# TAdeJong/pyGPA

Hardware: AMD Instinct MI355X
Metric: Mpixels/s displacement-field extraction (3 peaks, 4096^2 img) + achieved HBM GB/s (higher is better)
Workload: dtype f32; 1 GPU; 4096x4096 synthetic hex moire, 3 Bragg peaks x 16 k-vectors, sigma=10, weighted DCT-PCG unwrap kmax=10, image resident in HBM, u downloaded to pinned host memory inside the step (BASELINE.json configs[2]); x_planes=12, d2h_of_u=included, overlapped with the next step (copy stream), images_in_flight=1

## Files before the change

pygpa_amd/csrc/gpa_api.hip:

```cpp
#include "gpa_plan.h"

static thread_local std::string g_err;
int gpa_fail(int code, const std::string& msg) {
  g_err = msg;
  return code;
}
namespace gpa {
static const char* const kOptNames[OPT_COUNT] = {
    "PBS_FULLBAND", "SERIAL_UNWRAP", "NO_WORKER", "NO_KSPLIT", "NO_COMPACT", "NO_SHARED",
    "NO_PAIR", "TRI_SMALL", "TRI_Q", "NO_MR", "MR_FORCE_BLUESTEIN", "NO_ROWPQ", "COLSOLVE", "NO_LAT",
    "F32_EPS_FLOOR", "COLSTREAM_CHUNK", "NO_ROWHALF", "PAIR_MAXSIDE", "ROWHALF_MINLG", "NO_PQDCT",
    "NO_REORDER", "NO_RAW", "NO_TILEFUSE", "NO_ROWPERS", "NO_LFTILE", "LF_ALL_ROUNDS", "DFT_ENGINE", "GAUSS_FFT_MINR", "NO_GAUSS2D", "NO_DFT_HALF", "F32_STALL", "PBS_LDS_PAD", "NO_SHARED_PHASES", "PA_STAG", "PA_STAG_TICKS", "PA_ROT", "LF_STACK_BYTES", "NO_YSPEC", "YSPEC_GROUP", "NO_PB_SKIP"};
static OptVal g_opts[OPT_COUNT];
static std::once_flag g_opts_once;
static void opt_assign(OptVal& o, const char* value) {
  o.set = value != nullptr;
  o.num = value ? atof(value) : 0.0;
  memset(o.str, 0, sizeof(o.str));
  if (value) strncpy(o.str, value, sizeof(o.str) - 1);
}
static void opts_from_env() {
  for (int k = 0; k < OPT_COUNT; ++k) opt_assign(g_opts[k], getenv((std::string("GPA_") + kOptNames[k]).c_str()));
}
const OptVal& opt(OptKey k) {
  std::call_once(g_opts_once, opts_from_env);
  return g_opts[k];
}
}

Axis make_axis(int n) {
  Axis a;
  a.n = n;
  int lg = 0;
  while ((1 << lg) < n) ++lg;
  if ((1 << lg) == n) {
    a.padded = false;
  } else {
    lg = 0;
    while ((1 << lg) < 2 * n - 1) ++lg;
    a.padded = true;
  }
  if (lg < 6) {
    lg = 6;
    a.padded = ((1 << lg) != n);
  }
  a.lg = lg;
  a.L = 1 << lg;
  a.extL = a.padded ? n - 1 : 0;
  a.extR = 0;
  return a;
}

Axis compact_axis(const Axis& full, int E) {
  if (!full.padded || E >= (full.n - 1) / 2) return full;
  int lg = 6;
  while ((1 << lg) < full.n + 2 * E) ++lg;
  if (lg >= full.lg) return full;
  Axis a = full;
  a.lg = lg;
  a.L = 1 << lg;
  a.extL = a.extR = E;
  return a;
}

int upload_real_table(gpa_plan* p, void* dst, const std::vector<double>& v) {
  if (p->dtype == GPA_F32) HIP_TRY(upload_as<float>(dst, v, p->stream));
  else HIP_TRY(upload_as<double>(dst, v, p->stream));
  return GPA_OK;
}

int plan_reserve(gpa_plan* p, DevBuf& b, size_t bytes, const char* what) {
  const hipError_t e = b.reserve(bytes, p->stream);
  if (e != hipSuccess) return fail(GPA_ERR_HIP, std::string(what) + "(" + std::to_string(bytes) + "): " + hipGetErrorString(e));
  return GPA_OK;
}

int dmalloc(gpa_plan* p, void** ptr, size_t bytes) {
  DevBuf b(&p->ws_bytes);
  TRY(plan_reserve(p, b, bytes, "hipMalloc"));
  *ptr = b.ptr;
  p->owned.push_back(std::move(b));
  return GPA_OK;
}
int plan_build(gpa_plan* p) {
  HIP_TRY(hipSetDevice(p->device));
  HIP_TRY(hipStreamCreateWithFlags(&p->stream, hipStreamNonBlocking));
  HIP_TRY(hipEventCreate(&p->ev0));
  HIP_TRY(hipEventCreate(&p->ev1));
  for (auto& e : p->stage_ev) HIP_TRY(hipEventCreate(&e));
  const size_t npx = (size_t)p->n0 * p->n1;
  const int B = p->max_batch;
  TRY(dmalloc(p, &p->tw0, (size_t)p->ax0.L * p->csz));
  TRY(upload_twiddles(p, p->tw0, p->ax0.L));
  TRY(dmalloc(p, &p->tw1, (size_t)p->ax1.L * p->csz));
  TRY(upload_twiddles(p, p->tw1, p->ax1.L));
// ... 236 lines not shown
```

pygpa_amd/csrc/gpa_api_driver.hip:

```cpp
#include "gpa_plan.h"

struct ExtractOut {
  void* lockins;
  int32_t* kidx;
  void* grads;
  void* absw;
  int grad_mode;
};

static int check_ranges(gpa_plan* p, const std::string& fn, int P, int K, int kmax) {
  if (P < 2 || P > p->max_peaks) return fail(GPA_ERR_STATE, fn + ": need 2 <= P <= 8");
  if (K < 1 || P * K > p->max_batch) return fail(GPA_ERR_STATE, fn + ": P*K exceeds max_batch");
  if (kmax < 1) return fail(GPA_ERR_ARG, "kmax must be >= 1");
  return GPA_OK;
}

static int extract_stage(gpa_plan* p, const double* kvecs, int P, const double* klists, int K, double sigma, int* Bx, int passb) {
  TRY(stage_sweep(p, kvecs, P, klists, K, sigma, Bx, passb));
  TRY(stage_kmat(p, kvecs, P));
  {
    const size_t side = opt_set(OPT_PAIR_MAXSIDE) ? (size_t)opt(OPT_PAIR_MAXSIDE).num : 1024;
    p->use_pair = (size_t)p->n0 * p->n1 <= side * side && !opt_set(OPT_NO_PAIR);
  }
  if (p->use_pair && !p->have_uwp) {
// ... 185 lines not shown
                                         void* u, void* lockins, int32_t* kidx) {
  return extract_enqueue(p, "gpa_extract_displacement_field", image, kvecs, P, klists, K, sigma, mask_border, kmax, u,
                         {lockins, kidx, nullptr, nullptr, 0});
}

int gpa_extract_displacement_field_grad_async(gpa_plan* p, const void* image, const double* kvecs, int P,
                                              const double* klists, int K, double sigma, int mask_border, int kmax,
                                              int grad_mode, void* u, void* lockins, int32_t* kidx, void* grads, void* absw) {
  return extract_enqueue(p, "gpa_extract_displacement_field_grad_async", image, kvecs, P, klists, K, sigma, mask_border, kmax, u,
                         {lockins, kidx, grads, absw, grad_mode});
}

static int ensure_batch_unwrap(gpa_plan* p, int B) {
  if (B <= p->uwb_images) {
    if (!unwrap_set_active(&p->uwb, 2 * B)) return fail(GPA_ERR_STATE, "batched unwrap workspace: bad active count");
    return GPA_OK;
  }
  HIP_TRY(hipStreamSynchronize(p->stream));
  if (p->uwb_images) unwrap_workspace_destroy(&p->uwb);
  p->uwb_images = 0;
  p->uwb_bytes = 0;
  size_t bb = 0;
  hipError_t e = unwrap_workspace_create(p->dtype, p->n0, p->n1, p->stream, &p->uwb, &bb, 2 * B);
  if (e != hipSuccess) {
    unwrap_workspace_destroy(&p->uwb);
    return fail(GPA_ERR_HIP, std::string("batched unwrap workspace: ") + hipGetErrorString(e));
  }
  if (!unwrap_supports_batch(&p->uwb)) {
    unwrap_workspace_destroy(&p->uwb);
    return fail(GPA_ERR_STATE, "gpa_extract_displacement_field_batch: this image shape has no batched unwrap");
  }
  e = p->d_wnorm_b.reserve((size_t)B * p->n0 * p->n1 * p->rsz, p->stream);
  if (e == hipSuccess) e = p->h_iters_b.reserve((size_t)8 * B * sizeof(int), p->stream);
  if (e != hipSuccess) {
    unwrap_workspace_destroy(&p->uwb);
    return fail(GPA_ERR_HIP, std::string("batched driver buffers: ") + hipGetErrorString(e));
  }
  p->uwb_images = B;
  p->uwb_bytes = bb;
  return GPA_OK;
}

static int ensure_batch_sweep(gpa_plan* p, int chunk, size_t t_img, size_t l_img) {
  TRY(plan_reserve(p, p->bT, (size_t)chunk * t_img, "batched sweep buffers"));
  TRY(plan_reserve(p, p->bL, (size_t)chunk * l_img, "batched sweep buffers"));
  TRY(plan_reserve(p, p->bMean, (size_t)chunk * 8, "batched sweep buffers"));
  return plan_reserve(p, p->bScratch, (size_t)chunk * 1024 * sizeof(double), "batched sweep buffers");
}

static int read_batch_iters(gpa_plan* p, int B, int* iters_out) {
  HIP_TRY(hipStreamSynchronize(p->stream));
  for (int j = 0; j < 2 * B; ++j) iters_out[j] = p->h_iters_b.as<int>()[4 * j + unwrap_iters_slot(&p->uwb)];
  return GPA_OK;
}

int gpa_extract_displacement_field_batch_dev(gpa_plan* p, const void* images, int B, const double* kvecs, int P,
                                             const double* klists, int K, double sigma, int mask_border, int kmax,
                                             void* u, int* iters_out) {
  const char* fn = "gpa_extract_displacement_field_batch";
  if (!p || !images || !kvecs || !klists || !u) return fail(GPA_ERR_ARG, std::string(fn) + ": null argument");
  if (B < 1 || B > 4096) return fail(GPA_ERR_ARG, std::string(fn) + ": need 1 <= images <= 4096");
  TRY(check_ranges(p, fn, P, K, kmax));
  HIP_TRY(hipSetDevice(p->device));
  int Bx = 0;
  TRY(extract_stage(p, kvecs, P, klists, K, sigma, &Bx, SWEEP_PASSB_SELECT));
  TRY(ensure_batch_unwrap(p, B));
  const size_t npx = (size_t)p->n0 * p->n1;
  const size_t t_img = (size_t)Bx * npx * p->csz, l_img = (size_t)P * npx * p->csz;
  const int chunk = (int)std::min<size_t>((size_t)B, std::max<size_t>(1, ((size_t)3 << 30) / t_img));
  TRY(ensure_batch_sweep(p, chunk, t_img, l_img));
  int nparts = 0;
  const size_t rstride = 2 * npx;
  const size_t pstride = (size_t)(unwrap_partials_buffer(&p->uwb, 2) - unwrap_partials_buffer(&p->uwb, 0));
  for (int c0 = 0; c0 < B; c0 += chunk) {
    const int nimg = std::min(chunk, B - c0);
    const void* image = (const char*)images + (size_t)c0 * npx * p->rsz;
    HIP_TRY(launch_mean(p->dtype, image, npx, p->bScratch.as<double>(), p->bMean.ptr, p->stream, nimg));
    TRY(run_passA(p, image, p->bMean.ptr, p->bT.ptr, Bx, nimg));
    TRY(passB_select(p, {p->bT.ptr, nimg, Bx}, P, K, p->bL.ptr, nullptr, true));
    HIP_TRY(launch_reconstruct_setup(p->dtype, p->bL.ptr, p->d_kmat, P, p->n0, p->n1, mask_border,
                                     p->d_wnorm_b.as<char>() + (size_t)c0 * npx * p->rsz,
                                     unwrap_residual_buffer(&p->uwb, 2 * c0), unwrap_residual_buffer(&p->uwb, 2 * c0 + 1),
                                     unwrap_partials_buffer(&p->uwb, 2 * c0), unwrap_partials_buffer(&p->uwb, 2 * c0 + 1),
                                     &nparts, p->stream, nimg, rstride, pstride, p->lk_raw ? p->d_ystep : nullptr));
  }
  hipError_t e = unwrap_enqueue_prepared(&p->uwb, p->d_wnorm_b.ptr, nparts, kmax, 1e-9, true, u, p->stream);
  if (e == hipSuccess) e = unwrap_fetch_iters(&p->uwb, p->h_iters_b.as<int>(), p->stream);
  if (e != hipSuccess) return fail(GPA_ERR_HIP, std::string("batched unwrap: ") + hipGetErrorString(e));
  return iters_out ? read_batch_iters(p, B, iters_out) : GPA_OK;
}

int gpa_supports_batch(gpa_plan* p) {
  if (!p) return 0;
  return unwrap_supports_batch(&p->uw) ? 1 : 0;
}

int gpa_last_batch_iters(gpa_plan* p, int B, int* iters_out) {
  if (!p || !iters_out || B < 1 || B > p->uwb_images) return fail(GPA_ERR_ARG, "gpa_last_batch_iters: bad argument");
  return read_batch_iters(p, B, iters_out);
}

int gpa_extract_gradients(gpa_plan* p, const void* image, const double* kvecs, int P, const double* klists, int K,
                          double sigma, int mask_border, void* dudx, void* dudy, void* wnorm) {
  if (!p || !image || !kvecs || !klists || !dudx || !dudy || !wnorm)
    return fail(GPA_ERR_ARG, "gpa_extract_gradients: null argument");
  TRY(check_ranges(p, "gpa_extract_gradients", P, K, 1));
  HIP_TRY(hipSetDevice(p->device));
  const size_t npx = (size_t)p->n0 * p->n1;
  HIP_TRY(hipMemcpyAsync(p->d_image, image, npx * p->rsz, hipMemcpyHostToDevice, p->stream));
  TRY(sweep_peaks_dev(p, p->d_image, nullptr, kvecs, P, klists, K, sigma, p->d_lockin, nullptr, true));
  TRY(stage_kmat(p, kvecs, P));
  HIP_TRY(launch_reconstruct(p->dtype, p->d_lockin, p->d_kmat, P, p->n0, p->n1, mask_border, p->d_dudx, p->d_dudy,
                             p->d_wnorm, p->stream, p->lk_raw ? p->d_ystep : nullptr));
  HIP_TRY(hipMemcpyAsync(dudx, p->d_dudx, (size_t)2 * p->n0 * (p->n1 - 1) * p->rsz, hipMemcpyDeviceToHost, p->stream));
  HIP_TRY(hipMemcpyAsync(dudy, p->d_dudy, (size_t)2 * (p->n0 - 1) * p->n1 * p->rsz, hipMemcpyDeviceToHost, p->stream));
  HIP_TRY(hipMemcpyAsync(wnorm, p->d_wnorm, npx * p->rsz, hipMemcpyDeviceToHost, p->stream));
  HIP_TRY(hipStreamSynchronize(p->stream));
  return GPA_OK;
}
```

pygpa_amd/csrc/gpa_internal.h:

```cpp
#pragma once
#include <hip/hip_runtime.h>
#include <stdint.h>

#include "gpa_devbuf.h"
#include "gpa_fft.h"
#include "gpa_mrfft.h"

#ifndef GPA_F64_WAVES
#define GPA_F64_WAVES 2
#endif

namespace gpa {

struct KernelProfiler {
  struct Rec { const char* name; hipEvent_t a, b; };
  static constexpr int MAXREC = 4096;
  Rec rec[MAXREC];
  int n = 0;
  hipEvent_t pool[2 * MAXREC];
  int npool = 0;
};
extern thread_local KernelProfiler* g_kprof;
struct ProfScope {
  hipStream_t s;
  KernelProfiler::Rec* r = nullptr;
  ProfScope(const char* name, hipStream_t stream) : s(stream) {
    KernelProfiler* k = g_kprof;
    if (!k || k->n >= KernelProfiler::MAXREC) return;
    for (int j = 0; j < 2; ++j)
      if (k->npool < 2 * (k->n + 1)) { if (hipEventCreate(&k->pool[k->npool]) != hipSuccess) return; ++k->npool; }
    r = &k->rec[k->n];
    r->name = name;
    r->a = k->pool[2 * k->n];
    r->b = k->pool[2 * k->n + 1];
    ++k->n;
    (void)hipEventRecord(r->a, s);
  }
  ~ProfScope() { if (r) (void)hipEventRecord(r->b, s); }
};
#if defined(__HIPCC__)
__device__ __forceinline__ int xcd_tile(int b, int grid) {
  const int base = grid >> 3, rem = grid & 7, x = b & 7, idx = b >> 3;
  return x * base + (x < rem ? x : rem) + idx;
}
#endif

inline hipError_t set_dynamic_lds_once(const void* kern, int bytes, unsigned& done) {
  int dev = 0;
  (void)hipGetDevice(&dev);
  const unsigned bit = 1u << (dev & 31);
  if (done & bit) return hipSuccess;
  hipError_t e = hipFuncSetAttribute(kern, hipFuncAttributeMaxDynamicSharedMemorySize, bytes);
  if (e == hipSuccess) done |= bit;
  return e;
}

inline int device_cus() {
  static int n[32] = {};
  int dev = 0;
  (void)hipGetDevice(&dev);
  int& slot = n[dev & 31];
  if (!slot) {
    int cus = 0;
    if (hipDeviceGetAttribute(&cus, hipDeviceAttributeMultiprocessorCount, dev) != hipSuccess || cus <= 0) cus = 256;
    slot = cus;
  }
  return slot;
}

enum OptKey {
  OPT_PBS_FULLBAND, OPT_SERIAL_UNWRAP, OPT_NO_WORKER, OPT_NO_KSPLIT, OPT_NO_COMPACT, OPT_NO_SHARED,
  OPT_NO_PAIR, OPT_TRI_SMALL, OPT_TRI_Q, OPT_NO_MR, OPT_MR_FORCE_BLUESTEIN, OPT_NO_ROWPQ,
  OPT_COLSOLVE, OPT_NO_LAT, OPT_F32_EPS_FLOOR, OPT_COLSTREAM_CHUNK, OPT_NO_ROWHALF, OPT_PAIR_MAXSIDE, OPT_ROWHALF_MINLG, OPT_NO_PQDCT,
  OPT_NO_REORDER, OPT_NO_RAW, OPT_NO_TILEFUSE, OPT_NO_ROWPERS, OPT_NO_LFTILE, OPT_LF_ALL_ROUNDS, OPT_DFT_ENGINE, OPT_GAUSS_FFT_MINR, OPT_NO_GAUSS2D, OPT_NO_DFT_HALF, OPT_F32_STALL, OPT_PBS_LDS_PAD, OPT_NO_SHARED_PHASES, OPT_PA_STAG, OPT_PA_STAG_TICKS, OPT_PA_ROT, OPT_LF_STACK_BYTES, OPT_NO_YSPEC, OPT_YSPEC_GROUP, OPT_NO_PB_SKIP, OPT_COUNT
};
struct OptVal {
  bool set;
  double num;
  char str[24];
};
const OptVal& opt(OptKey k);
inline bool opt_set(OptKey k) { return opt(k).set; }

#define GPA_PROF_CAT2(a, b) a##b
#define GPA_PROF_CAT(a, b) GPA_PROF_CAT2(a, b)
#define GPA_PROF(name, stream) ::gpa::ProfScope GPA_PROF_CAT(_gpa_prof_, __LINE__)(name, stream)

struct Axis {
  int n;
  int lg;
  int L;
  bool padded;
  int extL, extR;
};
inline int axis_tpf(const Axis& a) { return a.L / 16; }

GPA_HD int axis_src(int m, int n, int L, bool padded, int extL, int extR) {
  if (!padded) return m;
  if (m < n) return m;
  if (m < n + extR) return m - n;
  if (m >= L - extL) return m - L + n;
  return -1;
}

struct SweepTables {
  void* cxb;
  void* sx;
  void* wxw;
  void* wxr;
  void* cyb;
  void* sy;
  void* wyw;
  void* wyr;
  void* dx;
  void* dy;
  int* planeof;
};

hipError_t launch_tables(int dtype, const Axis& a0, const Axis& a1, const double* kl,
                         const double* kr, int B, const double* pw, int Bx, const SweepTables& tb,
                         hipStream_t s);
hipError_t launch_mean(int dtype, const void* image, size_t count, double* scratch,
                       void* mean_out, hipStream_t s, int nimg = 1);
hipError_t launch_passA(int dtype, const Axis& a0, int n1, const void* image, const void* mean,
                        const SweepTables& tb, const void* Hx, const void* tw0, void* Tbuf,
                        int Bx, hipStream_t s, int nimg = 1);
struct PassAYspec {
  void* Yhat;
  void* strips;
  const int* groups;
  const int* planes;
  int ngroups;
  unsigned blockmask;
  int E, Epad;
};
hipError_t launch_passA_yspec(int dtype, const Axis& a0, const Axis& a1, const void* image, const void* mean,
                              const SweepTables& tb, const void* Hx, const void* tw0, const void* tw1, void* Tbuf, int Bx,
                              const PassAYspec& ys, hipStream_t s, int nimg = 1);
hipError_t launch_passB(int dtype, const Axis& a1, int n0, const void* Tbuf, const void* Hy,
                        const void* tw1, const SweepTables& tb, int P, int K, bool select,
                        void* out, int32_t* kidx, hipStream_t s, int nimg = 1, int Bx = 0);
hipError_t launch_passB_ext(int dtype, const Axis& a1, int n0, const void* Tbuf, const void* Hy, const void* tw1,
                            const SweepTables& tb, int K, int mode, void* out, int32_t* kidx, const uint8_t* gate,
                            void* psi, hipStream_t s, int P = 1);
hipError_t launch_passB_split(int dtype, const Axis& a1, int n0, const void* Tbuf, const void* Hy, const void* tw1,
                              const SweepTables& tb, int P, int K, int ksplit, void* part, int32_t* pidx, void* out,
                              int32_t* kidx, hipStream_t s);
hipError_t launch_phasegrad(int dtype, const void* psi, int K, const int32_t* kidx, int n0, int n1, const double* kl,
                            const double* kr, int mode, void* grad, hipStream_t s, const double* ystep = nullptr, int P = 1);
int passA_cols(int dtype, int lg);
int spec_index_rt(int lg, int tid, int reg, int elems = 16);

hipError_t launch_reconstruct(int dtype, const void* lockin, const double* kmat ,
                              int P, int n0, int n1, int border, void* dudx, void* dudy,
                              void* wnorm, hipStream_t s, const double* ystep = nullptr );

hipError_t launch_reconstruct_tile(int dtype, const void* lockin, const double* kmat, int P, int n0, int n1, int border,
                                   int i0, int j0, int t0, int t1, void* const dx[2], size_t dx_pitch, void* const dy[2],
                                   size_t dy_pitch, void* const wn[2], size_t wn_pitch, hipStream_t s,
                                   const double* ystep = nullptr);
hipError_t launch_reconstruct_setup(int dtype, const void* lockin, const double* kmat, int P, int n0, int n1,
                                    int border, void* wnorm, void* r0, void* r1, double* part0, double* part1,
                                    int* nparts, hipStream_t s, int nimg = 1, size_t rstride = 0, size_t pstride = 0,
                                    const double* ystep = nullptr );

hipError_t launch_prediff(int dtype, const void* grads, const void* w, const double* kmat, int P, int n0, int n1,
                          void* dudx, void* dudy, void* wnorm, hipStream_t s);

hipError_t launch_wlstsq(int dtype, const void* b, const void* w, const double* kmat, int P, size_t npx,
                         void* out, hipStream_t s);

hipError_t launch_jacobian(int dtype, const void* grads, const void* w, const double* kmat, int P, size_t npx,
                           double nmperpixel, const double* dks , void* J, hipStream_t s);
hipError_t launch_cabs(int dtype, const void* z, size_t count, void* out, hipStream_t s);
hipError_t launch_props(int dtype, const void* jac, size_t npx, int add_identity, double refangle, double refscale,
                        int diff, void* out, hipStream_t s);

struct KerelskyArgs {
  double a0[4], x0[4], retry_cost;
  int max_nfev, has_a0;
};
hipError_t launch_kerelsky(int dtype, const void* jac, size_t npx, const KerelskyArgs& p, void* out, double* cost, hipStream_t s);

hipError_t launch_field_jacobian(int dtype, int nimg, int n0, int n1, const void* u, double nmperpixel, int add_identity, void* J,
                                 void* props, double refangle, double refscale, int diff, hipStream_t s);
hipError_t launch_phases_jacobian(int dtype, int n0, int n1, int P, const double* kvecs, const void* phases, const void* weights,
                                  double nmperpixel, int add_identity, void* J, void* props, double refangle, double refscale,
                                  int diff, hipStream_t s);
hipError_t launch_phys_props(int dtype, const void* jac, size_t npx, int add_identity, double refangle, double refscale, int diff,
                             double poisson_ratio, void* out, hipStream_t s);

int huber_sums_offset();
hipError_t launch_huber_moments(int dtype, const void* img, int n0, int n1, const double* coef, double cx, double cy,
                                double sx, double sy, double* scratch, hipStream_t s);

hipError_t launch_polar_crop(int dtype, const void* lockins, int P, int n0, int n1, int edge, void* psi, void* amp,
                             void* amax, hipStream_t s);
hipError_t launch_sqrt_norm(int dtype, const void* amp, int P, size_t npx, const void* amax, void* weight, hipStream_t s);
size_t huber_batch_stride();
hipError_t launch_huber_moments_batch(int dtype, const void* imgs, int P, int n0, int n1, const double* state, double cx,
                                      double cy, double sx, double sy, double* work, double* sums, hipStream_t s);

constexpr int PEAK_PARTS = 1024;
bool gauss2d_small_ok(int R);
hipError_t launch_gauss2d_small(int dtype, const void* in, void* out, int n0, int n1, const double* w, int R,
                                const void* minuend, hipStream_t s);
hipError_t launch_gauss1d(int dtype, const void* in, void* out, int n0, int n1, int axis, const double* w, int R,
                          const void* minuend, hipStream_t s);
hipError_t launch_localmax(int dtype, const void* smooth, int n0, int n1, double rel, double* part, double* thr,
                           int max_out, int* count, int32_t* coords, void* vals, hipStream_t s);

hipError_t launch_deconv_pack(int dtype, const void* data, int m0, int m1, int pad, void* Z, hipStream_t s);
hipError_t launch_deconv_filter(int dtype, void* Z, int n0, int n1, const double* gx, const double* gy, double balance,
                                hipStream_t s);
hipError_t launch_deconv_unpack(int dtype, const void* Z, int m0, int m1, int pad, void* out, hipStream_t s);

hipError_t launch_tile_sums(int dtype, const void* wins, size_t win_stride, size_t pitch, const int* rects_dev, int ntiles,
                            int max_rows, double* part, double* out, hipStream_t s);
int tile_sums_bands(int max_rows);
hipError_t launch_set_mean(int dtype, const double* sum, double scale, void* mean_out, hipStream_t s);
hipError_t launch_copy_fields(int dtype, const void* const* src, void* const* dst, const size_t* src_pitch,
                              const size_t* dst_pitch, const int* rows, const int* cols, int nf, hipStream_t s);
hipError_t launch_stitch(int dtype, const void* tiles, size_t slot_stride, size_t field_stride, size_t tile_pitch,
                         const int* table_dev, int ntiles, int t0, int t1, int nf, void* const* dst, const size_t* dst_pitch,
                         const int* dst_rows, const int* dst_cols, hipStream_t s);

struct WarpWs {
  DevBuf buf;
  DevBuf taps;
  int taps_dtype = -1;
};
hipError_t warp_reserve_undistort(int dtype, int n0, int n1, WarpWs* ws, hipStream_t s);
hipError_t warp_invert_u(int dtype, const void* d_u, int n0, int n1, double scale, int iters, int edge, int shift,
                         void* d_out, hipStream_t s, int mode, int nan_last, WarpWs* ws, const int* rects = nullptr, int nrect = 0);
hipError_t warp_image(int dtype, const void* d_img, const void* d_uinv, int n0, int n1, void* d_out, hipStream_t s, WarpWs* ws,
                      const int* rects = nullptr, int nrect = 0);
int warp_stack_chunk(int dtype, int n0, int n1, int B, int per_frame);
hipError_t warp_undistort_stack(int dtype, const void* d_frames, int B, const void* d_u, int per_frame, double scale, void* d_uinv,
                                int n0, int n1, void* d_out, hipStream_t s, WarpWs* ws);
hipError_t spline_coef_constant_f64(const double* d_in, int n0, int n1, double* d_tmp, double* d_out, hipStream_t s, WarpWs* ws);

struct UcellGeom {
  double ks[4], kinv[4], rmin[2], z;
  int rs0, rs1;
};
struct UcellWs {
  DevBuf buf;
// ... 43 lines not shown
```

pygpa_amd/csrc/gpa_reconstruct.hip:

```cpp
#include "gpa_internal.h"
#include "gpa_jacmath.h"

namespace gpa {

template <class T>
__device__ __forceinline__ T wrap_diff_plus_step(T d, T hi, T lo) {
  const T pi = Consts<T>::pi, two_pi = Consts<T>::two_pi;
  d = d >= pi ? d - two_pi : (d < -pi ? d + two_pi : d);
  T x = d + hi;
  x = x >= pi ? x - two_pi : (x < -pi ? x + two_pi : x);
  return x + lo;
}

template <class T> __device__ __forceinline__ double unwrap_turn_scale() {
  return (double)Consts<T>::two_pi / 6.28318530717958647692;
}

constexpr int MAXP = 8;
constexpr int REC_ROWS = 16;

struct TileOut {
  int on;
  int i0, j0, t0, t1;
  int wx, hy;
  void *dx0, *dx1, *dy0, *dy1, *w0, *w1;
  size_t dxp, dyp, wp;
};

template <class T, int P>
__global__ __launch_bounds__(256) void reconstruct_kernel(const cpx<T>* __restrict__ lockin,
                                                         const double* __restrict__ kmat, int n0, int n1,
                                                         int border, T* __restrict__ dudx, T* __restrict__ dudy,
                                                         T* __restrict__ wnorm, const double* __restrict__ ystep,
                                                         const TileOut tile) {
  const int y = blockIdx.x * 256 + threadIdx.x;
  const int x0 = blockIdx.y * REC_ROWS;
  const int x1 = x0 + REC_ROWS < n0 ? x0 + REC_ROWS : n0;
  const int lane = threadIdx.x & 63;
  const bool act = y < n1;
  const int yc = act ? y : n1 - 1;
  const size_t npx = (size_t)n0 * n1;
  const bool has_r = act && yc + 1 < n1;
  T k0[P], k1[P], cy[P], cyl[P];
#pragma unroll
  for (int p = 0; p < P; ++p) {
    k0[p] = (T)kmat[2 * p];
    k1[p] = (T)kmat[2 * p + 1];
    const double c = ystep ? ystep[p] * unwrap_turn_scale<T>() : 0.0;
    cy[p] = (T)c;
    cyl[p] = (T)(c - (double)cy[p]);
  }
  T phc[P], ampc[P], phn[P], ampn[P];
#pragma unroll
  for (int p = 0; p < P; ++p) {
    const cpx<T> c = lockin[p * npx + (size_t)x0 * n1 + yc];
    phc[p] = atan2(c.y, c.x);
    ampc[p] = sqrt(c.x * c.x + c.y * c.y);
    phn[p] = T(0);
    ampn[p] = T(0);
  }
  for (int x = x0; x < x1; ++x) {
    const size_t o = (size_t)x * n1 + yc;
    const bool has_d = x + 1 < n0;
    if (has_d) {
#pragma unroll
      for (int p = 0; p < P; ++p) {
        const cpx<T> c = lockin[p * npx + o + n1];
        phn[p] = atan2(c.y, c.x);
        ampn[p] = sqrt(c.x * c.x + c.y * c.y);
      }
    }
    const bool inside = x >= border && x < n0 - border && yc >= border && yc < n1 - border;
    const T mfac = (inside ? T(1) : T(0)) + T(1e-6);
    T w[P], bx[P], by[P];
    T wmax = T(0), wsq = T(0);
#pragma unroll
    for (int p = 0; p < P; ++p) {
      T phr = __shfl_down(phc[p], 1);
      if (lane == 63 && has_r) {
        const cpx<T> c = lockin[p * npx + o + 1];
        phr = atan2(c.y, c.x);
      }
      w[p] = ampc[p] * mfac;
      wsq += w[p] * w[p];
      wmax = w[p] > wmax ? w[p] : wmax;
      bx[p] = has_r ? (ystep ? wrap_diff_plus_step(phr - phc[p], cy[p], cyl[p]) : wrap_phase_diff(phr - phc[p])) : T(0);
      by[p] = has_d ? wrap_phase_diff(phn[p] - phc[p]) : T(0);
    }
    const int xi = x - tile.i0, yj = yc - tile.j0;
    const bool tin = tile.on && xi >= 0 && xi < tile.t0 && yj >= 0 && yj < tile.t1;
    if (act && (!tile.on || tin)) {
      if (!tile.on) {
        if (wnorm) wnorm[o] = sqrt(wsq);
      } else {
        const T wv = sqrt(wsq);
        ((T*)tile.w0)[(size_t)xi * tile.wp + yj] = wv;
        if (tile.w1) ((T*)tile.w1)[(size_t)xi * tile.wp + yj] = wv;
      }
      const T ws = wmax > T(0) ? T(1) / wmax : T(0);
      T a00 = 0, a01 = 0, a11 = 0, rx0 = 0, rx1 = 0, ry0 = 0, ry1 = 0;
#pragma unroll
      for (int p = 0; p < P; ++p) {
        const T wn = w[p] * ws, ww = wn * wn;
        a00 += ww * k0[p] * k0[p];
        a01 += ww * k0[p] * k1[p];
        a11 += ww * k1[p] * k1[p];
        rx0 += ww * k0[p] * bx[p];
        rx1 += ww * k1[p] * bx[p];
        ry0 += ww * k0[p] * by[p];
        ry1 += ww * k1[p] * by[p];
      }
      if (has_r && (!tile.on || yj < tile.wx)) {
        T s0, s1;
        solve2(a00, a01, a11, rx0, rx1, s0, s1);
        if (!tile.on) {
          const size_t ox = (size_t)x * (n1 - 1) + yc, plane = (size_t)n0 * (n1 - 1);
          dudx[ox] = s0;
          dudx[plane + ox] = s1;
        } else {
          ((T*)tile.dx0)[(size_t)xi * tile.dxp + yj] = s0;
          ((T*)tile.dx1)[(size_t)xi * tile.dxp + yj] = s1;
        }
      }
      if (has_d && (!tile.on || xi < tile.hy)) {
        T s0, s1;
        solve2(a00, a01, a11, ry0, ry1, s0, s1);
        if (!tile.on) {
          const size_t plane = (size_t)(n0 - 1) * n1;
          dudy[o] = s0;
          dudy[plane + o] = s1;
        } else {
          ((T*)tile.dy0)[(size_t)xi * tile.dyp + yj] = s0;
          ((T*)tile.dy1)[(size_t)xi * tile.dyp + yj] = s1;
        }
      }
    }
#pragma unroll
    for (int p = 0; p < P; ++p) { phc[p] = phn[p]; ampc[p] = ampn[p]; }
  }
}

constexpr int FUSED_ROWS = 32, FUSED_COLS = 62;

template <class T, int P>
__global__ __launch_bounds__(256) void reconstruct_setup_kernel(const cpx<T>* __restrict__ lockin,
                                                               const double* __restrict__ kmat, int n0, int n1,
                                                               int border, T* __restrict__ wnorm, T* __restrict__ r0,
                                                               T* __restrict__ r1, double* __restrict__ part0,
                                                               double* __restrict__ part1, int band, size_t rstride,
                                                               size_t pstride, const double* __restrict__ ystep) {
  {
    const size_t img = blockIdx.z, npx_ = (size_t)n0 * n1;
    lockin += img * P * npx_;
    wnorm += img * npx_;
    r0 += img * rstride;
    r1 += img * rstride;
    part0 += img * pstride;
    part1 += img * pstride;
  }
  const int lane = threadIdx.x & 63, wave = threadIdx.x >> 6;
  const int yw = (blockIdx.x * 4 + wave) * FUSED_COLS + lane - 1;
  const bool incol = yw >= 0 && yw < n1;
  const int yc = yw < 0 ? 0 : (yw >= n1 ? n1 - 1 : yw);
  const bool outcol = incol && lane >= 1 && lane <= FUSED_COLS;
  const int x0 = blockIdx.y * band;
  const int x1 = x0 + band < n0 ? x0 + band : n0;
  const int xs = x0 > 0 ? x0 - 1 : x0;
  const size_t npx = (size_t)n0 * n1;
  const bool has_r = incol && yw + 1 < n1;
  T k0[P], k1[P];
#pragma unroll
  for (int p = 0; p < P; ++p) { k0[p] = (T)kmat[2 * p]; k1[p] = (T)kmat[2 * p + 1]; }
  T cy[P], cyl[P];
#pragma unroll
  for (int p = 0; p < P; ++p) {
    const double c = ystep ? ystep[p] * unwrap_turn_scale<T>() : 0.0;
    cy[p] = (T)c;
    cyl[p] = (T)(c - (double)cy[p]);
  }
  auto mask_fac = [&](int x, int y) {
    const bool inside = x >= border && x < n0 - border && y >= border && y < n1 - border;
    return (inside ? T(1) : T(0)) + T(1e-6);
  };
  T phc[P], ampc[P], phn[P], ampn[P];
  T wsq_c = T(0);
#pragma unroll
  for (int p = 0; p < P; ++p) {
    const cpx<T> c = lockin[p * npx + (size_t)xs * n1 + yc];
    phc[p] = atan2(c.y, c.x);
    ampc[p] = sqrt(c.x * c.x + c.y * c.y);
    phn[p] = T(0);
    ampn[p] = T(0);
    const T w = ampc[p] * mask_fac(xs, yc);
    wsq_c += w * w;
  }
  T fyu0 = T(0), fyu1 = T(0);
  double sq0 = 0, sq1 = 0;
  for (int x = xs; x < x1; ++x) {
    const size_t o = (size_t)x * n1 + yc;
    const bool has_d = x + 1 < n0, outrow = x >= x0;
    T wsq_n = T(0);
    if (has_d) {
      const T mn = mask_fac(x + 1, yc);
#pragma unroll
      for (int p = 0; p < P; ++p) {
        const cpx<T> c = lockin[p * npx + o + n1];
        phn[p] = atan2(c.y, c.x);
        ampn[p] = sqrt(c.x * c.x + c.y * c.y);
        const T w = ampn[p] * mn;
        wsq_n += w * w;
      }
    }
    const T tc = sqrt(wsq_c), tn = sqrt(wsq_n);
    const T wwc = tc * tc, wwn = tn * tn;
    const T wwr = __shfl_down(wwc, 1);
    const T mfac = mask_fac(x, yc);
    T w[P], bx[P], by[P];
    T wmax = T(0);
#pragma unroll
    for (int p = 0; p < P; ++p) {
      const T phr = __shfl_down(phc[p], 1);
      w[p] = ampc[p] * mfac;
      wmax = w[p] > wmax ? w[p] : wmax;
      bx[p] = has_r ? (ystep ? wrap_diff_plus_step(phr - phc[p], cy[p], cyl[p]) : wrap_phase_diff(phr - phc[p])) : T(0);
      by[p] = has_d ? wrap_phase_diff(phn[p] - phc[p]) : T(0);
    }
    const T ws = wmax > T(0) ? T(1) / wmax : T(0);
    T a00 = 0, a01 = 0, a11 = 0, rx0 = 0, rx1 = 0, ry0 = 0, ry1 = 0;
#pragma unroll
    for (int p = 0; p < P; ++p) {
      const T wn = w[p] * ws, ww = wn * wn;
      a00 += ww * k0[p] * k0[p];
      a01 += ww * k0[p] * k1[p];
      a11 += ww * k1[p] * k1[p];
      rx0 += ww * k0[p] * bx[p];
      rx1 += ww * k1[p] * bx[p];
      ry0 += ww * k0[p] * by[p];
      ry1 += ww * k1[p] * by[p];
    }
    T fx0 = T(0), fx1 = T(0), fy0 = T(0), fy1 = T(0);
    if (outrow && has_r) {
      T s0, s1;
      solve2(a00, a01, a11, rx0, rx1, s0, s1);
      const T m = wwr < wwc ? wwr : wwc;
      fx0 = wrap_to_pi_fast(s0) * m;
      fx1 = wrap_to_pi_fast(s1) * m;
    }
    if (has_d) {
      T s0, s1;
      solve2(a00, a01, a11, ry0, ry1, s0, s1);
      const T m = wwn < wwc ? wwn : wwc;
      fy0 = wrap_to_pi_fast(s0) * m;
      fy1 = wrap_to_pi_fast(s1) * m;
    }
    const T fxl0 = __shfl_up(fx0, 1), fxl1 = __shfl_up(fx1, 1);
    if (outrow && outcol) {
      const T v0 = fx0 - fxl0 + fy0 - fyu0, v1 = fx1 - fxl1 + fy1 - fyu1;
      wnorm[o] = tc;
      r0[o] = v0;
      r1[o] = v1;
      sq0 += (double)v0 * (double)v0;
      sq1 += (double)v1 * (double)v1;
    }
    fyu0 = fy0;
    fyu1 = fy1;
    wsq_c = wsq_n;
#pragma unroll
    for (int p = 0; p < P; ++p) { phc[p] = phn[p]; ampc[p] = ampn[p]; }
  }
  __shared__ double sh[8];
#pragma unroll
  for (int off = 32; off > 0; off >>= 1) { sq0 += __shfl_down(sq0, off); sq1 += __shfl_down(sq1, off); }
  if (lane == 0) { sh[wave] = sq0; sh[4 + wave] = sq1; }
  __syncthreads();
  if (threadIdx.x == 0) {
    const int blk = blockIdx.y * gridDim.x + blockIdx.x;
    part0[blk] = ((sh[0] + sh[1]) + sh[2]) + sh[3];
    part1[blk] = ((sh[4] + sh[5]) + sh[6]) + sh[7];
  }
}

template <class T>
static hipError_t launch_reconstruct_setup_t(const void* lockin, const double* kmat, int P, int n0, int n1, int border,
                                             void* wnorm, void* r0, void* r1, double* part0, double* part1, int* nparts,
                                             hipStream_t s, int nimg, size_t rstride, size_t pstride, const double* ystep) {
  int band = FUSED_ROWS;
  const int gx = (n1 + 4 * FUSED_COLS - 1) / (4 * FUSED_COLS);
  while (band > 2 && gx * ((n0 + band - 1) / band) < 1024) band /= 2;
  dim3 grid(gx, (n0 + band - 1) / band, nimg);
  *nparts = (int)(grid.x * grid.y);
  GPA_PROF("reconstruct_setup_kernel", s);
#define RS_CASE(PP)                                                                                                   \
  case PP:                                                                                                            \
    reconstruct_setup_kernel<T, PP><<<grid, 256, 0, s>>>((const cpx<T>*)lockin, kmat, n0, n1, border, (T*)wnorm,       \
                                                         (T*)r0, (T*)r1, part0, part1, band, rstride, pstride, ystep); \
    break;
  switch (P) {
    RS_CASE(2) RS_CASE(3) RS_CASE(4) RS_CASE(5) RS_CASE(6) RS_CASE(7) RS_CASE(8)
    default: return hipErrorInvalidValue;
  }
#undef RS_CASE
  return hipGetLastError();
}

hipError_t launch_reconstruct_setup(int dtype, const void* lockin, const double* kmat, int P, int n0, int n1,
                                    int border, void* wnorm, void* r0, void* r1, double* part0, double* part1,
                                    int* nparts, hipStream_t s, int nimg, size_t rstride, size_t pstride, const double* ystep) {
  if (P > MAXP || P < 2) return hipErrorInvalidValue;
  return dtype == 0 ? launch_reconstruct_setup_t<float>(lockin, kmat, P, n0, n1, border, wnorm, r0, r1, part0, part1, nparts, s,
                                                        nimg, rstride, pstride, ystep)
                    : launch_reconstruct_setup_t<double>(lockin, kmat, P, n0, n1, border, wnorm, r0, r1, part0, part1, nparts, s,
                                                         nimg, rstride, pstride, ystep);
}

template <class T>
__global__ __launch_bounds__(256) void wlstsq_kernel(const T* __restrict__ b, const T* __restrict__ w,
                                                    const double* __restrict__ kmat, int P, size_t npx,
                                                    T* __restrict__ out) {
  const size_t o = (size_t)blockIdx.x * 256 + threadIdx.x;
  if (o >= npx) return;
  T wv[MAXP], wmax = T(0);
  for (int p = 0; p < P; ++p) { wv[p] = w[p * npx + o]; const T a = wv[p] < T(0) ? -wv[p] : wv[p]; wmax = a > wmax ? a : wmax; }
  const T ws = wmax > T(0) ? T(1) / wmax : T(0);
  T a00 = 0, a01 = 0, a11 = 0, r0 = 0, r1 = 0;
  for (int p = 0; p < P; ++p) {
    const T k0 = (T)kmat[2 * p], k1 = (T)kmat[2 * p + 1], wn = wv[p] * ws, ww = wn * wn, bv = b[p * npx + o];
    a00 += ww * k0 * k0; a01 += ww * k0 * k1; a11 += ww * k1 * k1;
    r0 += ww * k0 * bv; r1 += ww * k1 * bv;
  }
  T s0, s1;
  solve2(a00, a01, a11, r0, r1, s0, s1);
  out[o] = s0;
  out[npx + o] = s1;
}

template <class T>
__global__ __launch_bounds__(256) void prediff_kernel(const T* __restrict__ g, const T* __restrict__ w,
                                                     const double* __restrict__ kmat, int P, int n0, int n1,
                                                     T* __restrict__ dudx, T* __restrict__ dudy, T* __restrict__ wnorm) {
  const int y = blockIdx.x * 256 + threadIdx.x, x = blockIdx.y;
  if (y >= n1) return;
  const size_t npx = (size_t)n0 * n1, o = (size_t)x * n1 + y;
  T wv[MAXP], wmax = T(0), wsq = T(0);
  for (int p = 0; p < P; ++p) {
    wv[p] = w[p * npx + o];
    const T a = wv[p] < T(0) ? -wv[p] : wv[p];
    wmax = a > wmax ? a : wmax;
  }
  const T ws = wmax > T(0) ? T(1) / wmax : T(0);
  T a00 = 0, a01 = 0, a11 = 0, rx0 = 0, rx1 = 0, ry0 = 0, ry1 = 0;
  for (int p = 0; p < P; ++p) {
    const T k0 = (T)kmat[2 * p], k1 = (T)kmat[2 * p + 1], wn = wv[p] * ws, ww = wn * wn;
    const T bx = wrap_to_pi(g[2 * (p * npx + o)]), by = wrap_to_pi(g[2 * (p * npx + o) + 1]);
    wsq += wn * wn;
    a00 += ww * k0 * k0; a01 += ww * k0 * k1; a11 += ww * k1 * k1;
    rx0 += ww * k0 * bx; rx1 += ww * k1 * bx;
    ry0 += ww * k0 * by; ry1 += ww * k1 * by;
  }
  T s0, s1;
  if (y + 1 < n1) {
    solve2(a00, a01, a11, rx0, rx1, s0, s1);
    dudx[(size_t)x * (n1 - 1) + y] = s0;
    dudx[(size_t)n0 * (n1 - 1) + (size_t)x * (n1 - 1) + y] = s1;
  }
  if (x + 1 < n0) {
    solve2(a00, a01, a11, ry0, ry1, s0, s1);
    dudy[o] = s0;
    dudy[(size_t)(n0 - 1) * n1 + o] = s1;
  }
  if (wnorm) wnorm[o] = sqrt(wsq) * wmax;
}

hipError_t launch_prediff(int dtype, const void* grads, const void* w, const double* kmat, int P, int n0, int n1,
                          void* dudx, void* dudy, void* wnorm, hipStream_t s) {
  if (P > MAXP) return hipErrorInvalidValue;
  dim3 grid((n1 + 255) / 256, n0);
  if (dtype == 0)
    prediff_kernel<float><<<grid, 256, 0, s>>>((const float*)grads, (const float*)w, kmat, P, n0, n1, (float*)dudx,
                                               (float*)dudy, (float*)wnorm);
  else
    prediff_kernel<double><<<grid, 256, 0, s>>>((const double*)grads, (const double*)w, kmat, P, n0, n1, (double*)dudx,
                                                (double*)dudy, (double*)wnorm);
  return hipGetLastError();
}

hipError_t launch_wlstsq(int dtype, const void* b, const void* w, const double* kmat, int P, size_t npx, void* out,
                         hipStream_t s) {
  if (P > MAXP) return hipErrorInvalidValue;
  const unsigned grid = (unsigned)((npx + 255) / 256);
  if (dtype == 0)
    wlstsq_kernel<float><<<grid, 256, 0, s>>>((const float*)b, (const float*)w, kmat, P, npx, (float*)out);
  else
    wlstsq_kernel<double><<<grid, 256, 0, s>>>((const double*)b, (const double*)w, kmat, P, npx, (double*)out);
  return hipGetLastError();
}
// ... 207 lines not shown
```

Before: 3719 Mpixels/s.

## Rebalance reconstruct-setup bands to resident waves and prefetch next lockin row

```diff
diff --git a/pygpa_amd/csrc/gpa_api.hip b/pygpa_amd/csrc/gpa_api.hip
--- a/pygpa_amd/csrc/gpa_api.hip
+++ b/pygpa_amd/csrc/gpa_api.hip
@@ -10,7 +10,7 @@
     "PBS_FULLBAND", "SERIAL_UNWRAP", "NO_WORKER", "NO_KSPLIT", "NO_COMPACT", "NO_SHARED",
     "NO_PAIR", "TRI_SMALL", "TRI_Q", "NO_MR", "MR_FORCE_BLUESTEIN", "NO_ROWPQ", "COLSOLVE", "NO_LAT",
     "F32_EPS_FLOOR", "COLSTREAM_CHUNK", "NO_ROWHALF", "PAIR_MAXSIDE", "ROWHALF_MINLG", "NO_PQDCT",
-    "NO_REORDER", "NO_RAW", "NO_TILEFUSE", "NO_ROWPERS", "NO_LFTILE", "LF_ALL_ROUNDS", "DFT_ENGINE", "GAUSS_FFT_MINR", "NO_GAUSS2D", "NO_DFT_HALF", "F32_STALL", "PBS_LDS_PAD", "NO_SHARED_PHASES", "PA_STAG", "PA_STAG_TICKS", "PA_ROT", "LF_STACK_BYTES", "NO_YSPEC", "YSPEC_GROUP", "NO_PB_SKIP"};
+    "NO_REORDER", "NO_RAW", "NO_TILEFUSE", "NO_ROWPERS", "NO_LFTILE", "LF_ALL_ROUNDS", "DFT_ENGINE", "GAUSS_FFT_MINR", "NO_GAUSS2D", "NO_DFT_HALF", "F32_STALL", "PBS_LDS_PAD", "NO_SHARED_PHASES", "PA_STAG", "PA_STAG_TICKS", "PA_ROT", "LF_STACK_BYTES", "NO_YSPEC", "YSPEC_GROUP", "NO_PB_SKIP", "SETUP_BAND"};
 static OptVal g_opts[OPT_COUNT];
 static std::once_flag g_opts_once;
 static void opt_assign(OptVal& o, const char* value) {
diff --git a/pygpa_amd/csrc/gpa_api_driver.hip b/pygpa_amd/csrc/gpa_api_driver.hip
--- a/pygpa_amd/csrc/gpa_api_driver.hip
+++ b/pygpa_amd/csrc/gpa_api_driver.hip
@@ -291,7 +291,7 @@
                                      p->d_wnorm_b.as<char>() + (size_t)c0 * npx * p->rsz,
                                      unwrap_residual_buffer(&p->uwb, 2 * c0), unwrap_residual_buffer(&p->uwb, 2 * c0 + 1),
                                      unwrap_partials_buffer(&p->uwb, 2 * c0), unwrap_partials_buffer(&p->uwb, 2 * c0 + 1),
-                                     &nparts, p->stream, nimg, rstride, pstride, p->lk_raw ? p->d_ystep : nullptr));
+                                     &nparts, p->stream, nimg, rstride, pstride, p->lk_raw ? p->d_ystep : nullptr, chunk));
   }
   hipError_t e = unwrap_enqueue_prepared(&p->uwb, p->d_wnorm_b.ptr, nparts, kmax, 1e-9, true, u, p->stream);
   if (e == hipSuccess) e = unwrap_fetch_iters(&p->uwb, p->h_iters_b.as<int>(), p->stream);
diff --git a/pygpa_amd/csrc/gpa_internal.h b/pygpa_amd/csrc/gpa_internal.h
--- a/pygpa_amd/csrc/gpa_internal.h
+++ b/pygpa_amd/csrc/gpa_internal.h
@@ -72,7 +72,7 @@
   OPT_PBS_FULLBAND, OPT_SERIAL_UNWRAP, OPT_NO_WORKER, OPT_NO_KSPLIT, OPT_NO_COMPACT, OPT_NO_SHARED,
   OPT_NO_PAIR, OPT_TRI_SMALL, OPT_TRI_Q, OPT_NO_MR, OPT_MR_FORCE_BLUESTEIN, OPT_NO_ROWPQ,
   OPT_COLSOLVE, OPT_NO_LAT, OPT_F32_EPS_FLOOR, OPT_COLSTREAM_CHUNK, OPT_NO_ROWHALF, OPT_PAIR_MAXSIDE, OPT_ROWHALF_MINLG, OPT_NO_PQDCT,
-  OPT_NO_REORDER, OPT_NO_RAW, OPT_NO_TILEFUSE, OPT_NO_ROWPERS, OPT_NO_LFTILE, OPT_LF_ALL_ROUNDS, OPT_DFT_ENGINE, OPT_GAUSS_FFT_MINR, OPT_NO_GAUSS2D, OPT_NO_DFT_HALF, OPT_F32_STALL, OPT_PBS_LDS_PAD, OPT_NO_SHARED_PHASES, OPT_PA_STAG, OPT_PA_STAG_TICKS, OPT_PA_ROT, OPT_LF_STACK_BYTES, OPT_NO_YSPEC, OPT_YSPEC_GROUP, OPT_NO_PB_SKIP, OPT_COUNT
+  OPT_NO_REORDER, OPT_NO_RAW, OPT_NO_TILEFUSE, OPT_NO_ROWPERS, OPT_NO_LFTILE, OPT_LF_ALL_ROUNDS, OPT_DFT_ENGINE, OPT_GAUSS_FFT_MINR, OPT_NO_GAUSS2D, OPT_NO_DFT_HALF, OPT_F32_STALL, OPT_PBS_LDS_PAD, OPT_NO_SHARED_PHASES, OPT_PA_STAG, OPT_PA_STAG_TICKS, OPT_PA_ROT, OPT_LF_STACK_BYTES, OPT_NO_YSPEC, OPT_YSPEC_GROUP, OPT_NO_PB_SKIP, OPT_SETUP_BAND, OPT_COUNT
 };
 struct OptVal {
   bool set;
@@ -162,7 +162,8 @@
 hipError_t launch_reconstruct_setup(int dtype, const void* lockin, const double* kmat, int P, int n0, int n1,
                                     int border, void* wnorm, void* r0, void* r1, double* part0, double* part1,
                                     int* nparts, hipStream_t s, int nimg = 1, size_t rstride = 0, size_t pstride = 0,
-                                    const double* ystep = nullptr );
+                                    const double* ystep = nullptr ,
+                                    int nimg_geom = 0);
 
 hipError_t launch_prediff(int dtype, const void* grads, const void* w, const double* kmat, int P, int n0, int n1,
                           void* dudx, void* dudy, void* wnorm, hipStream_t s);
diff --git a/pygpa_amd/csrc/gpa_reconstruct.hip b/pygpa_amd/csrc/gpa_reconstruct.hip
--- a/pygpa_amd/csrc/gpa_reconstruct.hip
+++ b/pygpa_amd/csrc/gpa_reconstruct.hip
@@ -1,4 +1,5 @@
 #include "gpa_internal.h"
+#include "gpa_reconstruct_geom.h"
 #include "gpa_jacmath.h"
 
 namespace gpa {
@@ -140,14 +141,63 @@
   }
 }
 
-constexpr int FUSED_ROWS = 32, FUSED_COLS = 62;
-
+constexpr int FUSED_COLS = SETUP_COLS;
+
+template <class T>
+__device__ __forceinline__ T lockin_abs(const cpx<T>& c) { return sqrt(fma(c.x, c.x, c.y * c.y)); }
 template <class T, int P>
+__device__ __forceinline__ T weight_norm2(const T (&amp)[P], T m) {
+  const T w0 = amp[0] * m, w1 = amp[1] * m;
+  T s = fma(w0, w0, w1 * w1);
+#pragma unroll
+  for (int p = 2; p < P; ++p) {
+    const T w = amp[p] * m;
+    s = fma(w, w, s);
+  }
+  return s;
+}
+
+template <class T>
+__device__ __forceinline__ void solve2_pair(T a00, T a01, T a11, T rx0, T rx1, T ry0, T ry1, T& sx0, T& sx1, T& sy0, T& sy1) {
+  const T det = fma(a00, a11, -(a01 * a01)), tr = a00 + a11;
+  const T tiny = sizeof(T) == 4 ? T(1e-12) : T(1e-28);
+  const T inv = T(1) / det;
+  sx0 = fma(a11, rx0, -(a01 * rx1)) * inv;
+  sx1 = fma(a00, rx1, -(a01 * rx0)) * inv;
+  sy0 = fma(a11, ry0, -(a01 * ry1)) * inv;
+  sy1 = fma(a00, ry1, -(a01 * ry0)) * inv;
+  if (!(det > tiny * tr * tr)) {
+    const bool some = tr > T(0);
+    sx0 = some ? rx0 / tr : T(0);
+    sx1 = some ? rx1 / tr : T(0);
+    sy0 = some ? ry0 / tr : T(0);
+    sy1 = some ? ry1 / tr : T(0);
+  }
+}
+
+template <class T>
+__device__ __forceinline__ void wrap4_to_pi_fast(T& a, T& b, T& c, T& d) {
+  const T two_pi = Consts<T>::two_pi;
+  const bool fa = fabs(a) < two_pi, fb = fabs(b) < two_pi, fc = fabs(c) < two_pi, fd = fabs(d) < two_pi;
+  const T a0 = a, b0 = b, c0 = c, d0 = d;
+  a = wrap_phase_diff(a0);
+  b = wrap_phase_diff(b0);
+  c = wrap_phase_diff(c0);
+  d = wrap_phase_diff(d0);
+  if (!(fa && fb && fc && fd)) {
+    a = fa ? a : wrap_to_pi(a0);
+    b = fb ? b : wrap_to_pi(b0);
+    c = fc ? c : wrap_to_pi(c0);
+    d = fd ? d : wrap_to_pi(d0);
+  }
+}
+
+template <class T, int P, bool AHEAD>
 __global__ __launch_bounds__(256) void reconstruct_setup_kernel(const cpx<T>* __restrict__ lockin,
                                                                const double* __restrict__ kmat, int n0, int n1,
                                                                int border, T* __restrict__ wnorm, T* __restrict__ r0,
                                                                T* __restrict__ r1, double* __restrict__ part0,
-                                                               double* __restrict__ part1, int band, size_t rstride,
+                                                               double* __restrict__ part1, SetupGeom geo, size_t rstride,
                                                                size_t pstride, const double* __restrict__ ystep) {
   {
     const size_t img = blockIdx.z, npx_ = (size_t)n0 * n1;
@@ -163,8 +213,7 @@
   const bool incol = yw >= 0 && yw < n1;
   const int yc = yw < 0 ? 0 : (yw >= n1 ? n1 - 1 : yw);
   const bool outcol = incol && lane >= 1 && lane <= FUSED_COLS;
-  const int x0 = blockIdx.y * band;
-  const int x1 = x0 + band < n0 ? x0 + band : n0;
+  const int x0 = geo.first_row(blockIdx.y), x1 = geo.first_row(blockIdx.y + 1);
   const int xs = x0 > 0 ? x0 - 1 : x0;
   const size_t npx = (size_t)n0 * n1;
   const bool has_r = incol && yw + 1 < n1;
@@ -182,37 +231,66 @@
     const bool inside = x >= border && x < n0 - border && y >= border && y < n1 - border;
     return (inside ? T(1) : T(0)) + T(1e-6);
   };
-  T phc[P], ampc[P], phn[P], ampn[P];
+  auto row_of = [&](int x) { return (size_t)(x < n0 ? x : n0 - 1) * n1 + yc; };
+  T phc[P], ampc[P];
+  cpx<T> ahead[AHEAD ? P : 1];
   T wsq_c = T(0);
-#pragma unroll
-  for (int p = 0; p < P; ++p) {
-    const cpx<T> c = lockin[p * npx + (size_t)xs * n1 + yc];
-    phc[p] = atan2(c.y, c.x);
-    ampc[p] = sqrt(c.x * c.x + c.y * c.y);
-    phn[p] = T(0);
-    ampn[p] = T(0);
-    const T w = ampc[p] * mask_fac(xs, yc);
-    wsq_c += w * w;
-  }
+  {
+    const size_t os = row_of(xs), o1 = row_of(xs + 1);
+    cpx<T> c[P];
+#pragma unroll
+    for (int p = 0; p < P; ++p) c[p] = lockin[p * npx + os];
+    if (AHEAD) {
+#pragma unroll
+      for (int p = 0; p < P; ++p) ahead[p] = lockin[p * npx + o1];
+    }
+#pragma unroll
+    for (int p = 0; p < P; ++p) {
+      phc[p] = atan2(c[p].y, c[p].x);
+      ampc[p] = lockin_abs(c[p]);
+    }
+    wsq_c = weight_norm2(ampc, mask_fac(xs, yc));
+  }
+  T tc = sqrt(wsq_c);
+  T wwc = tc * tc;
   T fyu0 = T(0), fyu1 = T(0);
   double sq0 = 0, sq1 = 0;
   for (int x = xs; x < x1; ++x) {
     const size_t o = (size_t)x * n1 + yc;
     const bool has_d = x + 1 < n0, outrow = x >= x0;
+    T phn[P], ampn[P];
     T wsq_n = T(0);
-    if (has_d) {
-      const T mn = mask_fac(x + 1, yc);
+    auto next_row = [&](const cpx<T>* cn) {
 #pragma unroll
       for (int p = 0; p < P; ++p) {
-        const cpx<T> c = lockin[p * npx + o + n1];
-        phn[p] = atan2(c.y, c.x);
-        ampn[p] = sqrt(c.x * c.x + c.y * c.y);
-        const T w = ampn[p] * mn;
-        wsq_n += w * w;
-      }
-    }
-    const T tc = sqrt(wsq_c), tn = sqrt(wsq_n);
-    const T wwc = tc * tc, wwn = tn * tn;
+        phn[p] = atan2(cn[p].y, cn[p].x);
+        ampn[p] = lockin_abs(cn[p]);
+      }
+      wsq_n = weight_norm2(ampn, mask_fac(x + 1, yc));
+    };
+    if constexpr (AHEAD) {
+      cpx<T> cn[P];
+#pragma unroll
+      for (int p = 0; p < P; ++p) cn[p] = ahead[p];
+      if (x + 1 < x1) {
+        const size_t o2 = row_of(x + 2);
+#pragma unroll
+        for (int p = 0; p < P; ++p) ahead[p] = lockin[p * npx + o2];
+      }
+      next_row(cn);
+      if (!has_d) wsq_n = T(0);
+    } else {
+#pragma unroll
+      for (int p = 0; p < P; ++p) { phn[p] = T(0); ampn[p] = T(0); }
+      if (has_d) {
+        cpx<T> cn[P];
+#pragma unroll
+        for (int p = 0; p < P; ++p) cn[p] = lockin[p * npx + o + n1];
+        next_row(cn);
+      }
+    }
+    const T tn = sqrt(wsq_n);
+    const T wwn = tn * tn;
     const T wwr = __shfl_down(wwc, 1);
     const T mfac = mask_fac(x, yc);
     T w[P], bx[P], by[P];
@@ -238,21 +316,13 @@
       ry0 += ww * k0[p] * by[p];
       ry1 += ww * k1[p] * by[p];
     }
-    T fx0 = T(0), fx1 = T(0), fy0 = T(0), fy1 = T(0);
-    if (outrow && has_r) {
-      T s0, s1;
-      solve2(a00, a01, a11, rx0, rx1, s0, s1);
-      const T m = wwr < wwc ? wwr : wwc;
-      fx0 = wrap_to_pi_fast(s0) * m;
-      fx1 = wrap_to_pi_fast(s1) * m;
-    }
-    if (has_d) {
-      T s0, s1;
-      solve2(a00, a01, a11, ry0, ry1, s0, s1);
-      const T m = wwn < wwc ? wwn : wwc;
-      fy0 = wrap_to_pi_fast(s0) * m;
-      fy1 = wrap_to_pi_fast(s1) * m;
-    }
+    T sx0, sx1, sy0, sy1;
+    solve2_pair(a00, a01, a11, rx0, rx1, ry0, ry1, sx0, sx1, sy0, sy1);
+    wrap4_to_pi_fast(sx0, sx1, sy0, sy1);
+    const T mx = wwr < wwc ? wwr : wwc, my = wwn < wwc ? wwn : wwc;
+    const bool ex = outrow && has_r;
+    const T fx0 = ex ? sx0 * mx : T(0), fx1 = ex ? sx1 * mx : T(0);
+    const T fy0 = has_d ? sy0 * my : T(0), fy1 = has_d ? sy1 * my : T(0);
     const T fxl0 = __shfl_up(fx0, 1), fxl1 = __shfl_up(fx1, 1);
     if (outrow && outcol) {
       const T v0 = fx0 - fxl0 + fy0 - fyu0, v1 = fx1 - fxl1 + fy1 - fyu1;
@@ -264,7 +334,8 @@
     }
     fyu0 = fy0;
     fyu1 = fy1;
-    wsq_c = wsq_n;
+    tc = tn;
+    wwc = wwn;
 #pragma unroll
     for (int p = 0; p < P; ++p) { phc[p] = phn[p]; ampc[p] = ampn[p]; }
   }
@@ -280,37 +351,73 @@
   }
 }
 
+#ifdef GPA_SETUP_AHEAD
+template <class T, int P> constexpr bool setup_ahead() { return GPA_SETUP_AHEAD != 0; }
+#else
+template <class T, int P> constexpr bool setup_ahead() { return sizeof(T) == 4 && P <= 3; }
+#endif
+
+template <class T, int P>
+static hipError_t setup_resident(int* out) {
+  static int n[32] = {};
+  int dev = 0;
+  (void)hipGetDevice(&dev);
+  int& slot = n[dev & 31];
+  if (!slot) {
+    int per_cu = 0;
+    const hipError_t e =
+        hipOccupancyMaxActiveBlocksPerMultiprocessor(&per_cu, reconstruct_setup_kernel<T, P, setup_ahead<T, P>()>, 256, 0);
+    if (e != hipSuccess) return e;
+    slot = (per_cu > 0 ? per_cu : 1) * device_cus();
+  }
+  *out = slot;
+  return hipSuccess;
+}
+
+template <class T, int P>
+static hipError_t launch_reconstruct_setup_p(const void* lockin, const double* kmat, int n0, int n1, int border, void* wnorm,
+                                             void* r0, void* r1, double* part0, double* part1, int* nparts, hipStream_t s,
+                                             int nimg, size_t rstride, size_t pstride, const double* ystep, int nimg_geom) {
+  int resident = 0;
+  const hipError_t e = setup_resident<T, P>(&resident);
+  if (e != hipSuccess) return e;
+  const int forced = opt_set(OPT_SETUP_BAND) && opt(OPT_SETUP_BAND).num >= 1 ? (int)opt(OPT_SETUP_BAND).num : 0;
+  const SetupGeom geo = setup_geometry(n0, n1, nimg_geom > nimg ? nimg_geom : nimg, resident, forced);
+  if (geo.bands < 1) return hipErrorInvalidValue;
+  dim3 grid(geo.gx, geo.bands, nimg);
+  *nparts = geo.gx * geo.bands;
+  GPA_PROF("reconstruct_setup_kernel", s);
+  reconstruct_setup_kernel<T, P, setup_ahead<T, P>()><<<grid, 256, 0, s>>>((const cpx<T>*)lockin, kmat, n0, n1, border,
+                                                                         (T*)wnorm, (T*)r0, (T*)r1, part0, part1, geo,
+                                                                         rstride, pstride, ystep);
+  return hipGetLastError();
+}
+
 template <class T>
 static hipError_t launch_reconstruct_setup_t(const void* lockin, const double* kmat, int P, int n0, int n1, int border,
                                              void* wnorm, void* r0, void* r1, double* part0, double* part1, int* nparts,
-                                             hipStream_t s, int nimg, size_t rstride, size_t pstride, const double* ystep) {
-  int band = FUSED_ROWS;
-  const int gx = (n1 + 4 * FUSED_COLS - 1) / (4 * FUSED_COLS);
-  while (band > 2 && gx * ((n0 + band - 1) / band) < 1024) band /= 2;
-  dim3 grid(gx, (n0 + band - 1) / band, nimg);
-  *nparts = (int)(grid.x * grid.y);
-  GPA_PROF("reconstruct_setup_kernel", s);
-#define RS_CASE(PP)                                                                                                   \
-  case PP:                                                                                                            \
-    reconstruct_setup_kernel<T, PP><<<grid, 256, 0, s>>>((const cpx<T>*)lockin, kmat, n0, n1, border, (T*)wnorm,       \
-                                                         (T*)r0, (T*)r1, part0, part1, band, rstride, pstride, ystep); \
-    break;
+                                             hipStream_t s, int nimg, size_t rstride, size_t pstride, const double* ystep,
+                                             int nimg_geom) {
+#define RS_CASE(PP)                                                                                                      \
+  case PP:                                                                                                               \
+    return launch_reconstruct_setup_p<T, PP>(lockin, kmat, n0, n1, border, wnorm, r0, r1, part0, part1, nparts, s, nimg, \
+                                             rstride, pstride, ystep, nimg_geom);
   switch (P) {
     RS_CASE(2) RS_CASE(3) RS_CASE(4) RS_CASE(5) RS_CASE(6) RS_CASE(7) RS_CASE(8)
     default: return hipErrorInvalidValue;
   }
 #undef RS_CASE
-  return hipGetLastError();
 }
 
 hipError_t launch_reconstruct_setup(int dtype, const void* lockin, const double* kmat, int P, int n0, int n1,
                                     int border, void* wnorm, void* r0, void* r1, double* part0, double* part1,
-                                    int* nparts, hipStream_t s, int nimg, size_t rstride, size_t pstride, const double* ystep) {
+                                    int* nparts, hipStream_t s, int nimg, size_t rstride, size_t pstride, const double* ystep,
+                                    int nimg_geom) {
   if (P > MAXP || P < 2) return hipErrorInvalidValue;
   return dtype == 0 ? launch_reconstruct_setup_t<float>(lockin, kmat, P, n0, n1, border, wnorm, r0, r1, part0, part1, nparts, s,
-                                                        nimg, rstride, pstride, ystep)
+                                                        nimg, rstride, pstride, ystep, nimg_geom)
                     : launch_reconstruct_setup_t<double>(lockin, kmat, P, n0, n1, border, wnorm, r0, r1, part0, part1, nparts, s,
-                                                         nimg, rstride, pstride, ystep);
+                                                         nimg, rstride, pstride, ystep, nimg_geom);
 }
 
 template <class T>
diff --git a/pygpa_amd/csrc/gpa_reconstruct_geom.h b/pygpa_amd/csrc/gpa_reconstruct_geom.h
--- /dev/null
+++ b/pygpa_amd/csrc/gpa_reconstruct_geom.h
@@ -0,0 +1,61 @@
+#pragma once
+
+#if defined(__HIPCC__)
+#define GPA_GEOM_HD __host__ __device__ inline
+#else
+#define GPA_GEOM_HD inline
+#endif
+
+namespace gpa {
+
+constexpr int SETUP_COLS = 62;
+constexpr int SETUP_ROWS = 32;
+constexpr int SETUP_ROWS_CAP = 64;
+constexpr int SETUP_MIN_GRID = 1024;
+constexpr int SETUP_MAXPART = 65536;
+
+struct SetupGeom {
+  int gx = 0;
+  int bands = 0;
+  int n0 = 0;
+  int fixed = 0;
+  GPA_GEOM_HD int first_row(int i) const {
+    if (fixed > 0) {
+      const long long x = (long long)i * fixed;
+      return x < n0 ? (int)x : n0;
+    }
+    return (int)((long long)i * n0 / bands);
+  }
+};
+
+inline int setup_ceil_div(long long a, long long b) { return (int)((a + b - 1) / b); }
+
+inline SetupGeom setup_geometry(int n0, int n1, int nimg, int resident, int forced_band = 0) {
+  SetupGeom g;
+  g.n0 = n0;
+  g.gx = setup_ceil_div(n1, 4 * SETUP_COLS);
+  if (n0 < 1 || n1 < 1 || nimg < 1) return g;
+  const long long per = (long long)g.gx * nimg;
+  if (per > SETUP_MAXPART) return g;
+  const int most = (int)(SETUP_MAXPART / per);
+  if (resident < 1) resident = 1;
+  int band = forced_band > 0 ? forced_band : SETUP_ROWS;
+  if (forced_band <= 0)
+    while (band > 2 && (long long)g.gx * setup_ceil_div(n0, band) < SETUP_MIN_GRID) band /= 2;
+  if (forced_band > 0 || band < SETUP_ROWS) {
+    while (setup_ceil_div(n0, band) > most) band *= 2;
+    g.fixed = band;
+    g.bands = setup_ceil_div(n0, band);
+    return g;
+  }
+  const int fewest = setup_ceil_div(n0, SETUP_ROWS_CAP);
+  const long long k = (per * fewest + resident - 1) / resident;
+  long long bands = k * resident / per;
+  if (bands > n0 / 2) bands = n0 / 2;
+  if (bands > most) bands = most;
+  if (bands < 1) bands = 1;
+  g.bands = (int)bands;
+  return g;
+}
+
+}
```

Result: no change. 3683 Mpixels/s (-1.0%).
